# salemon/quattro-transformer-ilqr

Measured on AMD Instinct MI355X. Metric: iLQR iterations/sec (batch x horizon steps/s), quadrotor N=50 batch=4096, higher is better.
Workload: dtype f32; 1 GPU; quadrotor n_x=12 n_u=4 N=50, pure iLQR iteration = simulate (nominal rollout + cost) + linearisation and Riccati sweep (one fused launch) + 6-alpha line search/commit (BASELINE configs[2]; configs[3] when n_gpus=8); batch_per_gpu=4096, global_batch=4096, horizon=50, n_x=12, n_u=4, integrator=euler, parallelism=dp1 (independent trajectory shards)

## Files before the change

### quattro-transformer-ilqr_amd/csrc/rollout_quad.hip

```cpp
#include "rollout_quad_body.h"

namespace {

template <bool RK4>
__global__ __launch_bounds__(64) void simulate_quad_kernel(const quattro_model_params p, const float* __restrict__ x0,
                                                           const float* __restrict__ u, int B, int N,
                                                           float* __restrict__ x, double* __restrict__ cost) {
  const int gid = blockIdx.x * blockDim.x + threadIdx.x;
  simulate_quad_body<RK4>(p, x0, u, N, x, cost, gid, (gid >> 2) < B);
}

template <bool RK4>
__global__ __launch_bounds__(64) void rollout_quad_kernel(const quattro_model_params p, const float* __restrict__ x_nom,
                                                          const float* __restrict__ u_nom, const float* __restrict__ K,
                                                          const float* __restrict__ k, AlphaList al, int n_alpha, int B,
                                                          int N, float* __restrict__ x_new, float* __restrict__ u_new,
                                                          double* __restrict__ cost, const int32_t* __restrict__ active) {
  const int gid = blockIdx.x * blockDim.x + threadIdx.x;
  const int b = gid >> 5, ai = (gid >> 2) & 7;
  const bool live = (b < B) && (active == nullptr || active[b < B ? b : 0] != 0);
  if (!__any(live)) return;
  const bool mine = live && ai < n_alpha;
  const size_t bb = live ? b : 0;
  const int aa = mine ? ai : 0;
  const LaneConst L = lane_const(p, gid & 3);
  const float* xn = x_nom + bb * (N + 1) * NX;
  const float* un = u_nom + bb * N * NU;
  const int wb = __builtin_amdgcn_readfirstlane(b);
  const NomSrc nom(L, x_nom, u_nom, K, k, N, wb, live ? b - wb : 0, 2);
  float alpha = al.a[0];
#pragma unroll
  for (int i = 1; i < QUATTRO_MAX_ALPHAS; ++i) alpha = (aa == i) ? al.a[i] : alpha;
  double J;
  if (x_new != nullptr && u_new != nullptr) {
    float* xo = x_new + ((size_t)aa * B + bb) * (N + 1) * NX;
    float* uo = u_new + ((size_t)aa * B + bb) * N * NU;
    if (mine && L.j < 3) {
#pragma unroll
      for (int g = 0; g < 4; ++g) xo[3 * g + L.a] = xn[3 * g + L.a];
    }
    J = quad_rollout_closed<RK4, 4, true>(p, L, nom, alpha, N, mine, ArrayStore(L, xo, uo, mine));
  } else {
    J = quad_rollout_closed<RK4, 4, true>(p, L, nom, alpha, N, mine, NoStore{});
  }
  J = quad_sum(J);
  if (mine && L.j == 0) cost[(size_t)ai * B + b] = J;
}

template <bool RK4>
__global__ __launch_bounds__(64) void linesearch_quad_kernel(const quattro_model_params p, float* x_nom, float* u_nom,
                                                             const float* __restrict__ K, const float* __restrict__ k,
                                                             AlphaList al, int n_alpha, int B, int N, double tol,
                                                             double* cost, int32_t* __restrict__ alpha_idx,
                                                             int32_t* active, int32_t* iters,
                                                             float* __restrict__ scratch) {
  linesearch_quad_body<RK4, 4, true>(p, x_nom, u_nom, K, k, al, n_alpha, B, N, tol, cost, alpha_idx, active, iters, scratch,
                                     blockIdx.x * blockDim.x + threadIdx.x, false);
}

}

#define QT_QUAD_DISPATCH(p, ...)                              \
  if ((p).integrator == QUATTRO_INTEGRATOR_EULER) {           \
    constexpr bool RK4 = false;                               \
    __VA_ARGS__;                                              \
  } else if ((p).integrator == QUATTRO_INTEGRATOR_RK4) {      \
    constexpr bool RK4 = true;                                \
    __VA_ARGS__;                                              \
  } else {                                                    \
    return QUATTRO_ERR_UNSUPPORTED;                           \
  }

int quattro_launch_simulate_quad(const quattro_model_params& p, const float* x0, const float* u, int B, int N, float* x,
                                 double* cost, hipStream_t stream) {
  const long long tot = (long long)B * 4;
  QT_QUAD_DISPATCH(p, hipLaunchKernelGGL((simulate_quad_kernel<RK4>), dim3((unsigned)((tot + 63) / 64)), dim3(64), 0,
                                         stream, p, x0, u, B, N, x, cost));
  return hipGetLastError() == hipSuccess ? QUATTRO_OK : QUATTRO_ERR_LAUNCH;
}

int quattro_launch_rollout_quad(const quattro_model_params& p, const float* x_nom, const float* u_nom, const float* K,
                                const float* k, const float* alphas, int n_alpha, int B, int N, float* x_new,
                                float* u_new, double* cost, const int32_t* active, hipStream_t stream) {
  AlphaList al;
  for (int i = 0; i < QUATTRO_MAX_ALPHAS; ++i) al.a[i] = i < n_alpha ? alphas[i] : 0.0f;
  const long long tot = (long long)B * 32;
  QT_QUAD_DISPATCH(p, hipLaunchKernelGGL((rollout_quad_kernel<RK4>), dim3((unsigned)((tot + 63) / 64)), dim3(64), 0,
                                         stream, p, x_nom, u_nom, K, k, al, n_alpha, B, N, x_new, u_new, cost, active));
  return hipGetLastError() == hipSuccess ? QUATTRO_OK : QUATTRO_ERR_LAUNCH;
}

int quattro_launch_linesearch_quad(const quattro_model_params& p, float* x_nom, float* u_nom, const float* K,
                                   const float* k, const float* alphas, int n_alpha, int B, int N, double tol,
                                   double* cost, int32_t* alpha_idx, int32_t* active, int32_t* iters, float* scratch,
                                   hipStream_t stream) {
  AlphaList al;
  for (int i = 0; i < QUATTRO_MAX_ALPHAS; ++i) al.a[i] = i < n_alpha ? alphas[i] : 0.0f;
  const long long tot = (long long)B * 32;
  QT_QUAD_DISPATCH(p, hipLaunchKernelGGL((linesearch_quad_kernel<RK4>), dim3((unsigned)((tot + 63) / 64)), dim3(64), 0,
                                         stream, p, x_nom, u_nom, K, k, al, n_alpha, B, N, tol, cost, alpha_idx, active,
                                         iters, scratch));
  return hipGetLastError() == hipSuccess ? QUATTRO_OK : QUATTRO_ERR_LAUNCH;
}
```

### quattro-transformer-ilqr_amd/csrc/rollout_quad_body.h

```cpp
#pragma once
#include "models_device.h"

namespace {

constexpr int NX = 12, NU = 4, CS = 16;

#define QT_QP(a, b, c, d) ((a) | ((b) << 2) | ((c) << 4) | ((d) << 6))
template <int CTRL>
__device__ __forceinline__ float quad_perm(float v) {
  return __builtin_bit_cast(float, __builtin_amdgcn_update_dpp(0, __builtin_bit_cast(int, v), CTRL, 0xf, 0xf, true));
}
template <int I>
__device__ __forceinline__ float quad_bcast(float v) {
  return quad_perm<QT_QP(I, I, I, I)>(v);
}
__device__ __forceinline__ double quad_sum(double v) {
  v += __shfl_xor(v, 1);
  v += __shfl_xor(v, 2);
  return v;
}

struct LaneConst {
  bool is0, is1;
  int a, j;
  float qw[4], qfw[4], xr[4];
  float rj;
  float tc[4];
  float gy, gz, inv_mass, dt;
  __device__ __forceinline__ float sel(float v0, float v1, float v2) const { return is0 ? v0 : (is1 ? v1 : v2); }
};

__device__ __forceinline__ LaneConst lane_const(const quattro_model_params& p, int j) {
  LaneConst L;
  L.j = j;
  L.a = j == 3 ? 0 : j;
  L.is0 = L.a == 0;
  L.is1 = L.a == 1;
  const float live = j == 3 ? 0.0f : 1.0f;
#pragma unroll
  for (int g = 0; g < 4; ++g) {
    L.qw[g] = live * L.sel(p.q[3 * g], p.q[3 * g + 1], p.q[3 * g + 2]);
    L.qfw[g] = live * L.sel(p.qf[3 * g], p.qf[3 * g + 1], p.qf[3 * g + 2]);
    L.xr[g] = L.sel(p.x_ref[3 * g], p.x_ref[3 * g + 1], p.x_ref[3 * g + 2]);
  }
  L.rj = p.r[j];
  const float Ix = p.phys[1], Iy = p.phys[2], Iz = p.phys[3], arm = p.phys[4], kyaw = p.phys[6];
  const float s0 = L.sel(-1.0f, 1.0f, 1.0f), s1 = L.sel(1.0f, 1.0f, -1.0f), s2 = L.sel(1.0f, -1.0f, 1.0f),
              s3 = L.sel(-1.0f, -1.0f, -1.0f);
  const float gain = L.sel(arm / Ix, arm / Iy, kyaw / Iz);
  L.tc[0] = s0 * gain; L.tc[1] = s1 * gain; L.tc[2] = s2 * gain; L.tc[3] = s3 * gain;
  L.gy = L.sel((Iy - Iz) / Ix, (Iz - Ix) / Iy, (Ix - Iy) / Iz);
  L.gz = L.sel(0.0f, 0.0f, -p.phys[5]);
  L.inv_mass = 1.0f / p.phys[0];
  L.dt = p.dt;
  return L;
}

struct QuadU {
  float u0, u1, u2, u3;
  __device__ __forceinline__ explicit QuadU(float uo)
      : u0(quad_bcast<0>(uo)), u1(quad_bcast<1>(uo)), u2(quad_bcast<2>(uo)), u3(quad_bcast<3>(uo)) {}
};

struct TrigBase {
  float a, s, c;
};
__device__ __forceinline__ void stage_sincos(const TrigBase& b, float x, float* s, float* c) {
  const float d = x - b.a;
  if (__builtin_expect(__any(!(fabsf(d) <= 0.25f)), 0)) {
    qt_sincos(x, s, c);
    return;
  }
  const float z = d * d;
  const float sd = d * fmaf(z, fmaf(z, fmaf(z, -1.9841270e-4f, 8.3333333e-3f), -1.6666667e-1f), 1.0f);
  const float cd = fmaf(z, fmaf(z, fmaf(z, -1.3888889e-3f, 4.1666667e-2f), -0.5f), 1.0f);
  *s = fmaf(b.s, cd, b.c * sd);
  *c = fmaf(b.c, cd, -(b.s * sd));
}

template <bool STAGE>
__device__ __forceinline__ void quad_rate(const LaneConst& L, const float* xo, const QuadU& U, float* xd, TrigBase& tb) {
  const float u0 = U.u0, u1 = U.u1, u2 = U.u2, u3 = U.u3;
  const float tm = (u0 + u1 + u2 + u3) * L.inv_mass;
  const float tau = fmaf(L.tc[3], u3, fmaf(L.tc[2], u2, fmaf(L.tc[1], u1, L.tc[0] * u0)));
  float so, co;
  if constexpr (STAGE) {
    stage_sincos(tb, xo[2], &so, &co);
  } else {
    qt_sincos_chain(xo[2], &so, &co);
    tb.a = xo[2]; tb.s = so; tb.c = co;
  }
  const float sph = quad_bcast<0>(so), cph = quad_bcast<0>(co), sth = quad_bcast<1>(so), cth = quad_bcast<1>(co),
              sps = quad_bcast<2>(so), cps = quad_bcast<2>(co);
  const float y = __builtin_amdgcn_rcpf(cth);
  const float sec = fmaf(fmaf(-cth, y, 1.0f), y, y);
  const float tth = sth * sec;
  const float wp = quad_bcast<0>(xo[3]), wq = quad_bcast<1>(xo[3]), wr = quad_bcast<2>(xo[3]);
  xd[0] = xo[1];
  const float ca = L.sel(sps, cps, 0.0f), cb = L.sel(cps * sth, -(sps * sth), cth);
  xd[1] = fmaf(tm, fmaf(ca, sph, cb * cph), L.gz);
  const float mix = fmaf(wq, sph, wr * cph);
  xd[2] = L.sel(fmaf(mix, tth, wp), fmaf(wq, cph, -(wr * sph)), mix * sec);
  xd[3] = fmaf(L.gy, L.sel(wq * wr, wp * wr, wp * wq), tau);
}

template <bool RK4>
__device__ __forceinline__ void quad_step(const LaneConst& L, const float* xo, const QuadU& uo, float* xn) {
  const float dt = L.dt;
  float k1[4];
  TrigBase tb;
  quad_rate<false>(L, xo, uo, k1, tb);
  if constexpr (!RK4) {
#pragma unroll
    for (int g = 0; g < 4; ++g) xn[g] = fmaf(dt, k1[g], xo[g]);
    return;
  }
  float k2[4], k3[4], k4[4], xs[4];
#pragma unroll
  for (int g = 0; g < 4; ++g) xs[g] = fmaf(0.5f * dt, k1[g], xo[g]);
  quad_rate<true>(L, xs, uo, k2, tb);
#pragma unroll
  for (int g = 0; g < 4; ++g) xs[g] = fmaf(0.5f * dt, k2[g], xo[g]);
  quad_rate<true>(L, xs, uo, k3, tb);
#pragma unroll
  for (int g = 0; g < 4; ++g) xs[g] = fmaf(dt, k3[g], xo[g]);
  quad_rate<true>(L, xs, uo, k4, tb);
#pragma unroll
  for (int g = 0; g < 4; ++g) xn[g] = xo[g] + (dt / 6.0f) * (k1[g] + 2.0f * k2[g] + 2.0f * k3[g] + k4[g]);
}

__device__ __forceinline__ float lane_stage_cost(const quattro_model_params& p, const LaneConst& L, const float* xo,
                                                 float uo, unsigned long long counted) {
  float c = 0.0f;
#pragma unroll
  for (int g = 0; g < 4; ++g) {
    const float d = xo[g] - L.xr[g];
    c = fmaf(L.qw[g] * d, d, c);
  }
  c = fmaf(L.rj * uo, uo, c);
  if (p.barrier_alpha != 0.0f) {
    const float ib = 1.0f / p.barrier_beta;
    const unsigned long long big = __builtin_amdgcn_ballot_w64(p.barrier_beta * uo > 20.0f);
    const unsigned long long tiny = __builtin_amdgcn_ballot_w64(fabsf(p.barrier_alpha) * 4.25e-18f * ib * ib < c * 2.9e-8f);
    if ((counted & ~(big & tiny)) != 0ull) {
      const float sp = qt_softplus(-uo, p.barrier_beta);
      c = fmaf(p.barrier_alpha, sp * sp, c);
    }
  }
  return c;
}

__device__ __forceinline__ float lane_final_cost(const LaneConst& L, const float* xo) {
  float c = 0.0f;
#pragma unroll
  for (int g = 0; g < 4; ++g) {
    const float d = xo[g] - L.xr[g];
    c = fmaf(L.qfw[g] * d, d, c);
  }
  return c;
}

struct NomSrc {
  __amdgpu_buffer_rsrc_t rx, ru, rK, rk;
  int vx, vu, vK;
  __device__ __forceinline__ NomSrc(const LaneConst& L, const float* x_nom, const float* u_nom, const float* K, const float* k,
                                    int N, int wb, int li, int nwt) {
    const size_t w = (size_t)wb;
    rx = __builtin_amdgcn_make_buffer_rsrc(const_cast<float*>(x_nom) + w * (N + 1) * NX, 0, nwt * (N + 1) * NX * 4, 0x00020000);
    ru = __builtin_amdgcn_make_buffer_rsrc(const_cast<float*>(u_nom) + w * N * NU, 0, nwt * N * NU * 4, 0x00020000);
    rK = __builtin_amdgcn_make_buffer_rsrc(const_cast<float*>(K) + w * N * NU * NX, 0, nwt * N * NU * NX * 4, 0x00020000);
    rk = __builtin_amdgcn_make_buffer_rsrc(const_cast<float*>(k) + w * N * NU, 0, nwt * N * NU * 4, 0x00020000);
    vx = 4 * (li * (N + 1) * NX + L.a);
    vu = 4 * (li * N * NU + L.j);
    vK = 4 * NX * (li * N * NU + L.j);
  }
};

struct NomLane {
  float x[4], u, k;
  float4 K[3];
  __device__ __forceinline__ void load(const NomSrc& s, int t) {
#pragma unroll
    for (int g = 0; g < 4; ++g) x[g] = __int_as_float(__builtin_amdgcn_raw_buffer_load_b32(s.rx, s.vx + 12 * g, t * (NX * 4), 0));
    u = __int_as_float(__builtin_amdgcn_raw_buffer_load_b32(s.ru, s.vu, t * (NU * 4), 0));
    k = __int_as_float(__builtin_amdgcn_raw_buffer_load_b32(s.rk, s.vu, t * (NU * 4), 0));
#pragma unroll
    for (int i = 0; i < 3; ++i) {
      const auto q = __builtin_amdgcn_raw_buffer_load_b128(s.rK, s.vK + 16 * i, t * (NU * NX * 4), 0);
      K[i] = make_float4(__int_as_float(q[0]), __int_as_float(q[1]), __int_as_float(q[2]), __int_as_float(q[3]));
    }
  }
};

__device__ __forceinline__ float4 gather_quarter(const LaneConst& L, const QuadU& U, const float* xn) {
  const float t0 = L.sel(xn[0], xn[1], xn[2]);
  const float t1 = quad_perm<QT_QP(1, 2, 0, 3)>(L.sel(xn[3], xn[0], xn[1]));
  const float t2 = quad_perm<QT_QP(2, 0, 1, 3)>(L.sel(xn[2], xn[3], xn[0]));
  const float t3 = L.sel(xn[1], xn[2], xn[3]);
  const bool l3 = L.j == 3;
  return make_float4(l3 ? U.u0 : t0, l3 ? U.u1 : t1, l3 ? U.u2 : t2, l3 ? U.u3 : t3);
}

struct NoStore {
  __device__ __forceinline__ void operator()(const LaneConst&, int, const QuadU&, const float*) const {}
};
struct ArrayStore {
  float* base;
  int stride;
  bool en;
  __device__ __forceinline__ ArrayStore(const LaneConst& L, float* xo, float* uo, bool en_)
      : base(L.j < 3 ? xo + NX + 4 * L.j : uo), stride(L.j < 3 ? NX : NU), en(en_) {}
  __device__ __forceinline__ void operator()(const LaneConst& L, int t, const QuadU& U, const float* xnext) const {
    const float4 v = gather_quarter(L, U, xnext);
    if (en) *reinterpret_cast<float4*>(base + (size_t)t * stride) = v;
  }
};
struct ScratchStore {
  float* s;
  bool en, l3;
  __device__ __forceinline__ ScratchStore(const LaneConst& L, float* rec, bool en_) : s(rec + 4 * L.j), en(en_), l3(L.j == 3) {}
  __device__ __forceinline__ void operator()(const LaneConst&, int t, const QuadU& U, const float* xnext) const {
    const float4 v = make_float4(l3 ? U.u0 : xnext[0], l3 ? U.u1 : xnext[1], l3 ? U.u2 : xnext[2], l3 ? U.u3 : xnext[3]);
    if (en) *reinterpret_cast<float4*>(s + (size_t)t * CS) = v;
  }
};

__device__ __forceinline__ float gain_dot(const float4* K, const float* dx, float acc) {
#define QT_FD(k, d, l) "v_fmac_f32_dpp %0, " d ", " k " quad_perm:[" l "," l "," l "," l "] row_mask:0xf bank_mask:0xf bound_ctrl:1\n\t"
  asm volatile("s_nop 1\n\t"
               QT_FD("%5", "%1", "0") QT_FD("%6", "%1", "1") QT_FD("%7", "%1", "2")
               QT_FD("%8", "%2", "0") QT_FD("%9", "%2", "1") QT_FD("%10", "%2", "2")
               QT_FD("%11", "%3", "0") QT_FD("%12", "%3", "1") QT_FD("%13", "%3", "2")
               QT_FD("%14", "%4", "0") QT_FD("%15", "%4", "1") QT_FD("%16", "%4", "2")
               : "+v"(acc)
               : "v"(dx[0]), "v"(dx[1]), "v"(dx[2]), "v"(dx[3]), "v"(K[0].x), "v"(K[0].y), "v"(K[0].z), "v"(K[0].w),
                 "v"(K[1].x), "v"(K[1].y), "v"(K[1].z), "v"(K[1].w), "v"(K[2].x), "v"(K[2].y), "v"(K[2].z), "v"(K[2].w));
#undef QT_FD
  return acc;
}

template <bool RK4, int PF, bool PRIO, class Store>
__device__ __forceinline__ double quad_rollout_closed(const quattro_model_params& p, const LaneConst& L,
                                                      const NomSrc& src, float alpha, int N, bool counted, Store store) {
  const unsigned long long counted_mask = __builtin_amdgcn_ballot_w64(counted);
  NomLane nb[PF];
#pragma unroll
  for (int d = 0; d < PF; ++d) nb[d].load(src, d < N ? d : N - 1);
  float xh[4];
#pragma unroll
  for (int g = 0; g < 4; ++g) xh[g] = nb[0].x[g];
  double J = 0.0;
  auto step = [&](const NomLane& b, int t) __attribute__((always_inline)) {
    if constexpr (PRIO) __builtin_amdgcn_s_setprio(1);
    float dx[4];
#pragma unroll
    for (int g = 0; g < 4; ++g) dx[g] = xh[g] - b.x[g];
    const float du = gain_dot(b.K, dx, b.k);
    const float uh = fmaf(alpha, du, b.u);
    if constexpr (!PRIO) J += (double)lane_stage_cost(p, L, xh, uh, counted_mask);
    float xnext[4];
    const QuadU U(uh);
    quad_step<RK4>(L, xh, U, xnext);
    if constexpr (PRIO) {
      __builtin_amdgcn_s_setprio(0);
      J += (double)lane_stage_cost(p, L, xh, uh, counted_mask);
    }
    store(L, t, U, xnext);
#pragma unroll
    for (int g = 0; g < 4; ++g) xh[g] = xnext[g];
  };
  int t = 0;
  for (; t + PF <= N; t += PF) {
#pragma unroll
    for (int d = 0; d < PF; ++d) {
      step(nb[d], t + d);
      nb[d].load(src, t + d + PF < N ? t + d + PF : N - 1);
    }
  }
#pragma unroll
  for (int d = 0; d < PF - 1; ++d)
    if (t + d < N) step(nb[d], t + d);
  J += (double)lane_final_cost(L, xh);
  return J;
}

template <bool RK4>
__device__ __forceinline__ void simulate_quad_body(const quattro_model_params& p, const float* __restrict__ x0,
                                                   const float* __restrict__ u, int N, float* __restrict__ x,
                                                   double* __restrict__ cost, const int gid, const bool live) {
  const int b = gid >> 2;
  const size_t bb = live ? b : 0;
  const LaneConst L = lane_const(p, gid & 3);
  const float* ub = u + bb * N * NU + L.j;
  float* xo = x + bb * (N + 1) * NX + L.a;
  float xh[4];
#pragma unroll
  for (int g = 0; g < 4; ++g) xh[g] = x0[bb * NX + 3 * g + L.a];
  const bool writer = live && L.j < 3;
  const int bw = __builtin_amdgcn_readfirstlane(b);
  const __amdgpu_buffer_rsrc_t rsx =
      __builtin_amdgcn_make_buffer_rsrc(x + (size_t)bw * (N + 1) * NX, 0, 16 * (N + 1) * NX * 4, 0x00020000);
  const int vox = writer ? 4 * ((b - bw) * (N + 1) * NX + L.a) : -1;
  if (writer) {
#pragma unroll
    for (int g = 0; g < 4; ++g) xo[3 * g] = xh[g];
  }
  double J = 0.0;
  const unsigned long long live_mask = __builtin_amdgcn_ballot_w64(live);
  float u0 = ub[0], u1 = ub[(size_t)(N > 1 ? 1 : 0) * NU];
  auto step = [&](float ut, int t) __attribute__((always_inline)) {
    J += (double)lane_stage_cost(p, L, xh, ut, live_mask);
    float xn[4];
    const QuadU U(ut);
    quad_step<RK4>(L, xh, U, xn);
#pragma unroll
    for (int g = 0; g < 4; ++g)
      __builtin_amdgcn_raw_buffer_store_b32(__float_as_int(xn[g]), rsx, vox, (t + 1) * (NX * 4) + 12 * g, 0);
#pragma unroll
    for (int g = 0; g < 4; ++g) xh[g] = xn[g];
  };
  asm volatile("" : "+v"(u0), "+v"(u1));
  __builtin_amdgcn_s_waitcnt(0x0f70);
  int t = 0;
  for (; t + 1 < N; t += 2) {
    step(u0, t);
    u0 = ub[(size_t)(t + 2 < N ? t + 2 : N - 1) * NU];
    step(u1, t + 1);
    u1 = ub[(size_t)(t + 3 < N ? t + 3 : N - 1) * NU];
  }
  if (t < N) step(u0, t);
  J += (double)lane_final_cost(L, xh);
  J = quad_sum(J);
  if (live && L.j == 0 && cost != nullptr) cost[b] = J;
}

template <bool RK4, int PF, bool PRIO>
__device__ __forceinline__ void linesearch_quad_body(const quattro_model_params& p, float* x_nom, float* u_nom,
                                                     const float* __restrict__ K, const float* __restrict__ k,
                                                     const AlphaList& al, int n_alpha, int B, int N, double tol,
                                                     double* cost, int32_t* __restrict__ alpha_idx, int32_t* active,
                                                     int32_t* iters, float* __restrict__ scratch, const int gid,
                                                     const bool force) {
  const int b = gid >> 5, ai = (gid >> 2) & 7, l32 = gid & 31;
  const bool live = (b < B) && (force || active == nullptr || active[b < B ? b : 0] != 0);
  if (!__any(live)) return;
  const bool mine = live && ai < n_alpha;
  const size_t bb = live ? b : 0;
  const int aa = mine ? ai : 0;
  const LaneConst L = lane_const(p, gid & 3);
  float* xn = x_nom + bb * (N + 1) * NX;
  float* un = u_nom + bb * N * NU;
  const int wb = __builtin_amdgcn_readfirstlane(b);
  const NomSrc nom(L, x_nom, u_nom, K, k, N, wb, live ? b - wb : 0, 2);
  float* sc = scratch + (bb * 8) * (size_t)N * CS;
  float alpha = al.a[0];
#pragma unroll
  for (int i = 1; i < QUATTRO_MAX_ALPHAS; ++i) alpha = (aa == i) ? al.a[i] : alpha;
  const double J0 = live ? cost[bb] : 0.0;
  double J = quad_rollout_closed<RK4, PF, PRIO>(p, L, nom, alpha, N, mine, ScratchStore(L, sc + (size_t)aa * N * CS, mine));
  J = quad_sum(J);
  const bool ok = mine && (J <= J0);
  const unsigned long long bal = __ballot(ok);
  const int lane = threadIdx.x & 63;
  const unsigned grp = (unsigned)((bal >> (lane & 32)) & 0x11111111ull);
  const int first = grp ? ((__ffs((int)grp) - 1) >> 2) : -1;
  if (live && first >= 0) {
    __builtin_amdgcn_fence(__ATOMIC_RELEASE, "workgroup");
    asm volatile("s_waitcnt vmcnt(0)" ::: "memory");
    __builtin_amdgcn_fence(__ATOMIC_ACQUIRE, "workgroup");
    const float* src = sc + (size_t)first * N * CS;
    const int e = l32 & 15, half = l32 >> 4;
    const bool isx = e < 12;
    const int slot = isx ? 4 * (e % 3) + e / 3 : e;
    float* dst = isx ? xn + NX + e : un + (e - 12);
    const int dstride = isx ? NX : NU;
    constexpr int COPY_U = 13;
    for (int t0 = half; t0 < N; t0 += 2 * COPY_U) {
      float v[COPY_U];
#pragma unroll
      for (int q = 0; q < COPY_U; ++q) {
        const int t = t0 + 2 * q;
        v[q] = src[(size_t)(t < N ? t : t0) * CS + slot];
      }
#pragma unroll
      for (int q = 0; q < COPY_U; ++q) {
        const int t = t0 + 2 * q;
        if (t < N) dst[(size_t)t * dstride] = v[q];
      }
    }
    if (ai == first && L.j == 0) {
      cost[b] = J;
      if (active != nullptr && fabs(J0 - J) < tol) active[b] = 0;
    }
  }
  if (live && l32 == 0) {
    if (alpha_idx != nullptr) alpha_idx[b] = first;
    if (iters != nullptr) iters[b] += 1;
    if (first < 0 && active != nullptr) active[b] = 0;
  }
}

}
```

Baseline: 1.952 billion steps/s.

## Split line-search into producer/consumer wavefronts via an LDS ring buffer

The line-search kernel now launches two wavefronts per block. Wave 0 runs the closed-loop rollout at raised priority and pushes each step's state and control into a double-buffered shared-memory ring. Wave 1 reads the ring, accumulates stage and final costs, and writes the scratch records. The aim is to move the cost evaluation and the scratch stores off the serial dynamics recurrence so they overlap with it. The price is a workgroup barrier every 8 steps, more LDS per block, and twice the threads per trajectory, which may lower occupancy.

```diff
diff --git a/quattro-transformer-ilqr_amd/csrc/rollout_quad.hip b/quattro-transformer-ilqr_amd/csrc/rollout_quad.hip
--- a/quattro-transformer-ilqr_amd/csrc/rollout_quad.hip
+++ b/quattro-transformer-ilqr_amd/csrc/rollout_quad.hip
@@ -48,14 +48,15 @@
 }
 
 template <bool RK4>
-__global__ __launch_bounds__(64) void linesearch_quad_kernel(const quattro_model_params p, float* x_nom, float* u_nom,
-                                                             const float* __restrict__ K, const float* __restrict__ k,
-                                                             AlphaList al, int n_alpha, int B, int N, double tol,
-                                                             double* cost, int32_t* __restrict__ alpha_idx,
-                                                             int32_t* active, int32_t* iters,
-                                                             float* __restrict__ scratch) {
-  linesearch_quad_body<RK4, 4, true>(p, x_nom, u_nom, K, k, al, n_alpha, B, N, tol, cost, alpha_idx, active, iters, scratch,
-                                     blockIdx.x * blockDim.x + threadIdx.x, false);
+__global__ __launch_bounds__(128) void linesearch_quad_kernel(const quattro_model_params p, float* x_nom, float* u_nom,
+                                                              const float* __restrict__ K, const float* __restrict__ k,
+                                                              AlphaList al, int n_alpha, int B, int N, double tol,
+                                                              double* cost, int32_t* __restrict__ alpha_idx,
+                                                              int32_t* active, int32_t* iters,
+                                                              float* __restrict__ scratch) {
+  __shared__ Ring ring;
+  linesearch_quad_body<RK4, 4, false, true>(p, x_nom, u_nom, K, k, al, n_alpha, B, N, tol, cost, alpha_idx, active, iters,
+                                            scratch, blockIdx.x * 64 + (threadIdx.x & 63), false, &ring);
 }
 
 }
@@ -97,7 +98,7 @@
   AlphaList al;
   for (int i = 0; i < QUATTRO_MAX_ALPHAS; ++i) al.a[i] = i < n_alpha ? alphas[i] : 0.0f;
   const long long tot = (long long)B * 32;
-  QT_QUAD_DISPATCH(p, hipLaunchKernelGGL((linesearch_quad_kernel<RK4>), dim3((unsigned)((tot + 63) / 64)), dim3(64), 0,
+  QT_QUAD_DISPATCH(p, hipLaunchKernelGGL((linesearch_quad_kernel<RK4>), dim3((unsigned)((tot + 63) / 64)), dim3(128), 0,
                                          stream, p, x_nom, u_nom, K, k, al, n_alpha, B, N, tol, cost, alpha_idx, active,
                                          iters, scratch));
   return hipGetLastError() == hipSuccess ? QUATTRO_OK : QUATTRO_ERR_LAUNCH;
diff --git a/quattro-transformer-ilqr_amd/csrc/rollout_quad_body.h b/quattro-transformer-ilqr_amd/csrc/rollout_quad_body.h
--- a/quattro-transformer-ilqr_amd/csrc/rollout_quad_body.h
+++ b/quattro-transformer-ilqr_amd/csrc/rollout_quad_body.h
@@ -220,7 +220,9 @@
   bool en, l3;
   __device__ __forceinline__ ScratchStore(const LaneConst& L, float* rec, bool en_) : s(rec + 4 * L.j), en(en_), l3(L.j == 3) {}
   __device__ __forceinline__ void operator()(const LaneConst&, int t, const QuadU& U, const float* xnext) const {
-    const float4 v = make_float4(l3 ? U.u0 : xnext[0], l3 ? U.u1 : xnext[1], l3 ? U.u2 : xnext[2], l3 ? U.u3 : xnext[3]);
+    put(t, make_float4(l3 ? U.u0 : xnext[0], l3 ? U.u1 : xnext[1], l3 ? U.u2 : xnext[2], l3 ? U.u3 : xnext[3]));
+  }
+  __device__ __forceinline__ void put(int t, const float4& v) const {
     if (en) *reinterpret_cast<float4*>(s + (size_t)t * CS) = v;
   }
 };
@@ -239,9 +241,65 @@
   return acc;
 }
 
+constexpr int RING_R = 8;
+struct RingSlot {
+  float4 x[64];
+  float u[64];
+};
+struct Ring {
+  RingSlot s[2][RING_R];
+};
+__device__ __forceinline__ void ring_barrier() {
+  __builtin_amdgcn_fence(__ATOMIC_RELEASE, "workgroup", "local");
+  __builtin_amdgcn_s_barrier();
+  __builtin_amdgcn_fence(__ATOMIC_ACQUIRE, "workgroup", "local");
+}
+struct RingPut {
+  Ring* r;
+  int lane;
+  __device__ __forceinline__ void operator()(int t, float uh, const float* xnext) const {
+    RingSlot& s = r->s[(t / RING_R) & 1][t % RING_R];
+    s.x[lane] = make_float4(xnext[0], xnext[1], xnext[2], xnext[3]);
+    s.u[lane] = uh;
+  }
+  __device__ __forceinline__ void close(int N) const {
+    if (N % RING_R != 0) ring_barrier();
+  }
+};
+template <class Put>
+__device__ __forceinline__ double ring_cost(const quattro_model_params& p, const LaneConst& L, const Ring* r, int lane, int N,
+                                            bool counted, float* xh, Put put) {
+  const unsigned long long counted_mask = __builtin_amdgcn_ballot_w64(counted);
+  double J = 0.0;
+  for (int t0 = 0; t0 < N; t0 += RING_R) {
+    ring_barrier();
+    const RingSlot* blk = r->s[(t0 / RING_R) & 1];
+    float4 xb[RING_R];
+    float ub[RING_R];
+#pragma unroll
+    for (int i = 0; i < RING_R; ++i) {
+      xb[i] = blk[i].x[lane];
+      ub[i] = blk[i].u[lane];
+    }
+#pragma unroll
+    for (int i = 0; i < RING_R; ++i) {
+      if (t0 + i < N) {
+        const float4 xn = xb[i];
+        J += (double)lane_stage_cost(p, L, xh, ub[i], counted_mask);
+        put(t0 + i, blk[i], xn);
+        xh[0] = xn.x; xh[1] = xn.y; xh[2] = xn.z; xh[3] = xn.w;
+      }
+    }
+  }
+  J += (double)lane_final_cost(L, xh);
+  return J;
+}
+
 template <bool RK4, int PF, bool PRIO, class Store>
 __device__ __forceinline__ double quad_rollout_closed(const quattro_model_params& p, const LaneConst& L,
                                                       const NomSrc& src, float alpha, int N, bool counted, Store store) {
+  constexpr bool SPLIT = __is_same(Store, RingPut);
+  static_assert(!SPLIT || (RING_R % PF == 0 && !PRIO), "a block of the ring is a whole number of prefetch groups");
   const unsigned long long counted_mask = __builtin_amdgcn_ballot_w64(counted);
   NomLane nb[PF];
 #pragma unroll
@@ -257,7 +315,7 @@
     for (int g = 0; g < 4; ++g) dx[g] = xh[g] - b.x[g];
     const float du = gain_dot(b.K, dx, b.k);
     const float uh = fmaf(alpha, du, b.u);
-    if constexpr (!PRIO) J += (double)lane_stage_cost(p, L, xh, uh, counted_mask);
+    if constexpr (!PRIO && !SPLIT) J += (double)lane_stage_cost(p, L, xh, uh, counted_mask);
     float xnext[4];
     const QuadU U(uh);
     quad_step<RK4>(L, xh, U, xnext);
@@ -265,7 +323,10 @@
       __builtin_amdgcn_s_setprio(0);
       J += (double)lane_stage_cost(p, L, xh, uh, counted_mask);
     }
-    store(L, t, U, xnext);
+    if constexpr (SPLIT)
+      store(t, uh, xnext);
+    else
+      store(L, t, U, xnext);
 #pragma unroll
     for (int g = 0; g < 4; ++g) xh[g] = xnext[g];
   };
@@ -276,10 +337,16 @@
       step(nb[d], t + d);
       nb[d].load(src, t + d + PF < N ? t + d + PF : N - 1);
     }
+    if constexpr (SPLIT)
+      if ((t + PF) % RING_R == 0) ring_barrier();
   }
 #pragma unroll
   for (int d = 0; d < PF - 1; ++d)
     if (t + d < N) step(nb[d], t + d);
+  if constexpr (SPLIT) {
+    store.close(N);
+    return 0.0;
+  }
   J += (double)lane_final_cost(L, xh);
   return J;
 }
@@ -334,13 +401,13 @@
   if (live && L.j == 0 && cost != nullptr) cost[b] = J;
 }
 
-template <bool RK4, int PF, bool PRIO>
+template <bool RK4, int PF, bool PRIO, bool SPLIT = false>
 __device__ __forceinline__ void linesearch_quad_body(const quattro_model_params& p, float* x_nom, float* u_nom,
                                                      const float* __restrict__ K, const float* __restrict__ k,
                                                      const AlphaList& al, int n_alpha, int B, int N, double tol,
                                                      double* cost, int32_t* __restrict__ alpha_idx, int32_t* active,
                                                      int32_t* iters, float* __restrict__ scratch, const int gid,
-                                                     const bool force) {
+                                                     const bool force, Ring* ring = nullptr) {
   const int b = gid >> 5, ai = (gid >> 2) & 7, l32 = gid & 31;
   const bool live = (b < B) && (force || active == nullptr || active[b < B ? b : 0] != 0);
   if (!__any(live)) return;
@@ -357,11 +424,30 @@
 #pragma unroll
   for (int i = 1; i < QUATTRO_MAX_ALPHAS; ++i) alpha = (aa == i) ? al.a[i] : alpha;
   const double J0 = live ? cost[bb] : 0.0;
-  double J = quad_rollout_closed<RK4, PF, PRIO>(p, L, nom, alpha, N, mine, ScratchStore(L, sc + (size_t)aa * N * CS, mine));
+  const int lane = threadIdx.x & 63;
+  const ScratchStore store(L, sc + (size_t)aa * N * CS, mine);
+  double J;
+  if constexpr (SPLIT) {
+    if (__builtin_amdgcn_readfirstlane(threadIdx.x >> 6) == 0) {
+      __builtin_amdgcn_s_setprio(1);
+      quad_rollout_closed<RK4, PF, false>(p, L, nom, alpha, N, mine, RingPut{ring, lane});
+      return;
+    }
+    float xh[4];
+#pragma unroll
+    for (int g = 0; g < 4; ++g) xh[g] = __int_as_float(__builtin_amdgcn_raw_buffer_load_b32(nom.rx, nom.vx + 12 * g, 0, 0));
+    asm volatile("" : "+v"(xh[0]), "+v"(xh[1]), "+v"(xh[2]), "+v"(xh[3]));
+    __builtin_amdgcn_s_waitcnt(0x0f70);
+    const int rec = L.j == 3 ? (int)sizeof(RingSlot::x) + 4 * (lane - 3) : 16 * lane;
+    J = ring_cost(p, L, ring, lane, N, mine, xh, [&](int t, const RingSlot& s, const float4&) {
+      store.put(t, *reinterpret_cast<const float4*>(reinterpret_cast<const char*>(&s) + rec));
+    });
+  } else {
+    J = quad_rollout_closed<RK4, PF, PRIO>(p, L, nom, alpha, N, mine, store);
+  }
   J = quad_sum(J);
   const bool ok = mine && (J <= J0);
   const unsigned long long bal = __ballot(ok);
-  const int lane = threadIdx.x & 63;
   const unsigned grp = (unsigned)((bal >> (lane & 32)) & 0x11111111ull);
   const int first = grp ? ((__ffs((int)grp) - 1) >> 2) : -1;
   if (live && first >= 0) {
```

Result: faster. 1.978 billion steps/s (median of 6 runs) (+1.3%).

## Add cascaded chunked simulate kernel splitting attitude chain from parallel position and cost work

Applied to the files above, without the earlier changes.

Adds a new Euler-only simulate kernel that handles 8 trajectories per 256-thread block and processes the horizon in chunks of 64 steps. Within each chunk, one wave runs only the serial attitude/angular-rate recurrence. The other threads then compute accelerations, stage costs and coalesced float4 state stores in parallel, using shared memory as the staging area. The aim is to shorten the serial dependency chain of the nominal rollout and improve parallelism and store coalescing. The cost is extra shared memory, several block-wide barriers per chunk, and a fallback to the old kernel when pointers are not 16-byte aligned.

```diff
diff --git a/quattro-transformer-ilqr_amd/csrc/rollout_quad.hip b/quattro-transformer-ilqr_amd/csrc/rollout_quad.hip
--- a/quattro-transformer-ilqr_amd/csrc/rollout_quad.hip
+++ b/quattro-transformer-ilqr_amd/csrc/rollout_quad.hip
@@ -1,4 +1,5 @@
 #include "rollout_quad_body.h"
+#include "simulate_cascade_body.h"
 
 namespace {
 
@@ -73,6 +74,11 @@
 
 int quattro_launch_simulate_quad(const quattro_model_params& p, const float* x0, const float* u, int B, int N, float* x,
                                  double* cost, hipStream_t stream) {
+  if (p.integrator == QUATTRO_INTEGRATOR_EULER && (((uintptr_t)u | (uintptr_t)x) & 15) == 0) {
+    hipLaunchKernelGGL(simulate_cascade_kernel, dim3((unsigned)(((long long)B + CAS_TPB - 1) / CAS_TPB)), dim3(CAS_THREADS),
+                       0, stream, p, x0, u, B, N, x, cost);
+    return hipGetLastError() == hipSuccess ? QUATTRO_OK : QUATTRO_ERR_LAUNCH;
+  }
   const long long tot = (long long)B * 4;
   QT_QUAD_DISPATCH(p, hipLaunchKernelGGL((simulate_quad_kernel<RK4>), dim3((unsigned)((tot + 63) / 64)), dim3(64), 0,
                                          stream, p, x0, u, B, N, x, cost));
diff --git a/quattro-transformer-ilqr_amd/csrc/simulate_cascade_body.h b/quattro-transformer-ilqr_amd/csrc/simulate_cascade_body.h
--- /dev/null
+++ b/quattro-transformer-ilqr_amd/csrc/simulate_cascade_body.h
@@ -0,0 +1,161 @@
+#pragma once
+#include "rollout_quad_body.h"
+
+namespace {
+
+constexpr int CAS_TPB = 8;
+constexpr int CAS_THREADS = 256;
+constexpr int CAS_TC = 64;
+constexpr int CAS_SLOTS = 4 * CAS_TPB;
+constexpr int CAS_RS = 4 * CAS_SLOTS + 4;
+constexpr int CAS_BLK = 8;
+static_assert(CAS_TC % CAS_BLK == 0, "a block of read-ahead rows must stay inside the chunk");
+
+__global__ __launch_bounds__(CAS_THREADS) void simulate_cascade_kernel(const quattro_model_params p,
+                                                                       const float* __restrict__ x0,
+                                                                       const float* __restrict__ u, int B, int N,
+                                                                       float* __restrict__ x, double* __restrict__ cost) {
+  __shared__ __attribute__((aligned(16))) float rec[(CAS_TC + 1) * CAS_RS];
+  __shared__ __attribute__((aligned(16))) float uL[CAS_TC * CAS_SLOTS];
+  __shared__ __attribute__((aligned(16))) float tauL[CAS_TC * CAS_SLOTS];
+  const int tid = threadIdx.x, lane = tid & 63, wave = tid >> 6;
+  const int slot = tid & (CAS_SLOTS - 1), tr = slot >> 2;
+  const int b0 = blockIdx.x * CAS_TPB;
+  const bool live = b0 + tr < B;
+  const size_t bb = live ? b0 + tr : b0;
+  const LaneConst L = lane_const(p, tid & 3);
+  const bool chain = tid < CAS_SLOTS;
+  float* const rp = rec + 4 * slot;
+  float xh[4] = {0.0f, 0.0f, 0.0f, 0.0f};
+  double J = 0.0;
+  if (chain) {
+#pragma unroll
+    for (int g = 0; g < 4; ++g) xh[g] = x0[bb * NX + 3 * g + L.a];
+  }
+  for (int t0 = 0; t0 < N; t0 += CAS_TC) {
+    const int n = N - t0 < CAS_TC ? N - t0 : CAS_TC;
+    {
+      const LaneConst A0 = lane_const(p, 0), A1 = lane_const(p, 1), A2 = lane_const(p, 2);
+      const int tj = tid & (CAS_TPB - 1);
+      const size_t bu = b0 + tj < B ? b0 + tj : b0;
+      for (int tt = tid / CAS_TPB; tt < n; tt += CAS_THREADS / CAS_TPB) {
+        const float4 uv = *reinterpret_cast<const float4*>(u + (bu * N + t0 + tt) * NU);
+        const float u0 = uv.x, u1 = uv.y, u2 = uv.z, u3 = uv.w;
+        const float ta = fmaf(A0.tc[3], u3, fmaf(A0.tc[2], u2, fmaf(A0.tc[1], u1, A0.tc[0] * u0)));
+        const float tb = fmaf(A1.tc[3], u3, fmaf(A1.tc[2], u2, fmaf(A1.tc[1], u1, A1.tc[0] * u0)));
+        const float tc = fmaf(A2.tc[3], u3, fmaf(A2.tc[2], u2, fmaf(A2.tc[1], u1, A2.tc[0] * u0)));
+        *reinterpret_cast<float4*>(uL + 4 * (tt * CAS_TPB + tj)) = uv;
+        *reinterpret_cast<float4*>(tauL + 4 * (tt * CAS_TPB + tj)) = make_float4(ta, tb, tc, ta);
+      }
+    }
+    __syncthreads();
+    if (chain) {
+      const float* tp = tauL + slot;
+      float ang = xh[2], om = xh[3];
+      for (int t = 0; t < n; ++t) {
+        const float tau = tp[t * CAS_SLOTS];
+        float so, co;
+        qt_sincos_chain(ang, &so, &co);
+        *reinterpret_cast<float4*>(rp + t * CAS_RS) = make_float4(so, co, ang, om);
+        const float sph = quad_bcast<0>(so), cph = quad_bcast<0>(co), sth = quad_bcast<1>(so), cth = quad_bcast<1>(co);
+        const float y = __builtin_amdgcn_rcpf(cth);
+        const float sec = fmaf(fmaf(-cth, y, 1.0f), y, y);
+        const float tth = sth * sec;
+        const float wp = quad_bcast<0>(om), wq = quad_bcast<1>(om), wr = quad_bcast<2>(om);
+        const float mix = fmaf(wq, sph, wr * cph);
+        const float da = L.sel(fmaf(mix, tth, wp), fmaf(wq, cph, -(wr * sph)), mix * sec);
+        const float dw = fmaf(L.gy, L.sel(wq * wr, wp * wr, wp * wq), tau);
+        ang = fmaf(L.dt, da, ang);
+        om = fmaf(L.dt, dw, om);
+      }
+      *reinterpret_cast<float2*>(rp + n * CAS_RS + 2) = make_float2(ang, om);
+      xh[2] = ang;
+      xh[3] = om;
+    }
+    __syncthreads();
+    for (int i = tid; i < n * CAS_SLOTS; i += CAS_THREADS) {
+      const int tt = i / CAS_SLOTS;
+      const float2 sc = *reinterpret_cast<const float2*>(rp + tt * CAS_RS);
+      const float so = sc.x, co = sc.y;
+      const float sph = quad_bcast<0>(so), cph = quad_bcast<0>(co), sth = quad_bcast<1>(so), cth = quad_bcast<1>(co),
+                  sps = quad_bcast<2>(so), cps = quad_bcast<2>(co);
+      const float4 uv = *reinterpret_cast<const float4*>(uL + 4 * (tt * CAS_TPB + tr));
+      const float tm = (uv.x + uv.y + uv.z + uv.w) * L.inv_mass;
+      const float ca = L.sel(sps, cps, 0.0f), cb = L.sel(cps * sth, -(sps * sth), cth);
+      rp[tt * CAS_RS] = fmaf(tm, fmaf(ca, sph, cb * cph), L.gz);
+    }
+    __syncthreads();
+    if (chain) {
+      float pa = xh[0], va = xh[1];
+      for (int tb = 0; tb < n; tb += CAS_BLK) {
+        float acc[CAS_BLK];
+#pragma unroll
+        for (int q = 0; q < CAS_BLK; ++q) acc[q] = rp[(tb + q) * CAS_RS];
+#pragma unroll
+        for (int q = 0; q < CAS_BLK; ++q) {
+          if (tb + q < n) {
+            *reinterpret_cast<float2*>(rp + (tb + q) * CAS_RS) = make_float2(pa, va);
+            pa = fmaf(L.dt, va, pa);
+            va = fmaf(L.dt, acc[q], va);
+          }
+        }
+      }
+      *reinterpret_cast<float2*>(rp + n * CAS_RS) = make_float2(pa, va);
+      xh[0] = pa;
+      xh[1] = va;
+    }
+    __syncthreads();
+    if (cost != nullptr) {
+      for (int i0 = wave * 64; i0 < n * CAS_SLOTS; i0 += CAS_THREADS) {
+        const int i = i0 + lane;
+        const bool valid = i < n * CAS_SLOTS;
+        const int tt = valid ? i / CAS_SLOTS : n - 1;
+        const float4 xv = *reinterpret_cast<const float4*>(rp + tt * CAS_RS);
+        const float xo[4] = {xv.x, xv.y, xv.z, xv.w};
+        const float c = lane_stage_cost(p, L, xo, uL[tt * CAS_SLOTS + slot], __builtin_amdgcn_ballot_w64(valid && live));
+        if (valid) tauL[tt * CAS_SLOTS + slot] = c;
+      }
+    }
+    {
+      const int r0 = t0 == 0 ? 0 : 1;
+      const int items = 3 * (n + 1 - r0);
+#pragma unroll
+      for (int k = 0; k < CAS_TPB / 4; ++k) {
+        const int tj = wave + 4 * k;
+        if (b0 + tj >= B) continue;
+        float* dst = x + ((size_t)(b0 + tj) * (N + 1) + t0 + r0) * NX;
+        for (int i = lane; i < items; i += 64) {
+          const int r = r0 + i / 3, q = i % 3;
+          float v[4];
+#pragma unroll
+          for (int e = 0; e < 4; ++e) {
+            const int s = 4 * q + e;
+            v[e] = rec[r * CAS_RS + 4 * (4 * tj + s % 3) + s / 3];
+          }
+          *reinterpret_cast<float4*>(dst + 4 * i) = make_float4(v[0], v[1], v[2], v[3]);
+        }
+      }
+    }
+    if (cost != nullptr) {
+      __syncthreads();
+      if (chain) {
+        for (int tb = 0; tb < n; tb += CAS_BLK) {
+          float c[CAS_BLK];
+#pragma unroll
+          for (int q = 0; q < CAS_BLK; ++q) c[q] = tauL[(tb + q) * CAS_SLOTS + slot];
+#pragma unroll
+          for (int q = 0; q < CAS_BLK; ++q)
+            if (tb + q < n) J += (double)c[q];
+        }
+      }
+    }
+    if (t0 + CAS_TC < N) __syncthreads();
+  }
+  if (cost != nullptr && wave == 0) {
+    if (chain) J += (double)lane_final_cost(L, xh);
+    J = quad_sum(J);
+    if (chain && live && L.j == 0) cost[b0 + tr] = J;
+  }
+}
+
+}
```

Result: slower. 1.943 billion steps/s before, 1.824 billion steps/s after, median of 2 (-6.2%).
